# zovoilis-lab/Flye

Hardware: AMD Instinct MI355X
Metric: Gbp reads overlapped/sec (higher is better)
Workload: dtype u64

## Files before the change

flye_amd/csrc/fg_api.hip:

```cpp
#include "fg_ctx.h"
#include "fg_stage.h"
#include <chrono>
#include <cmath>

#include <algorithm>
#include <new>

#include <mutex>
#include <atomic>

static std::mutex g_poolMutex;
static std::vector<BatchOwner*> g_pool;

BatchOwner* BatchOwner::acquire()
{
	std::lock_guard<std::mutex> lock(g_poolMutex);
	if (g_pool.empty()) return new BatchOwner;
	BatchOwner* b = g_pool.back();
	g_pool.pop_back();
	return b;
}

void BatchOwner::release(BatchOwner* b)
{
// ... 39 lines not shown
	}
}

const char* fg_last_error(const fg_ctx* ctx) { return ctx ? ctx->lastError.c_str() : ""; }

int fg_create(fg_ctx** out, int device, int kmer_size)
{
	if (!out) return FG_ERR_ARG;
	*out = nullptr;
	if (kmer_size < 1 || kmer_size > 32) return FG_ERR_KMER_SIZE;
	RandStreamGuard keepCallersRandStream;
	int count = 0;
	if (hipGetDeviceCount(&count) != hipSuccess || count <= 0) return FG_ERR_NO_DEVICE;
	if (device < 0 || device >= count) return FG_ERR_NO_DEVICE;
	if (hipSetDevice(device) != hipSuccess) return FG_ERR_NO_DEVICE;
	fg_ctx* c = new (std::nothrow) fg_ctx;
	if (!c) return FG_ERR_NOMEM;
	c->device = device;
	c->k = kmer_size;
	if (hipStreamCreateWithFlags(&c->stream, hipStreamNonBlocking) != hipSuccess ||
		hipStreamCreateWithFlags(&c->stream2, hipStreamNonBlocking) != hipSuccess ||
		hipStreamCreateWithFlags(&c->stream3, hipStreamNonBlocking) != hipSuccess ||
		hipEventCreateWithFlags(&c->evJoin3, hipEventDisableTiming) != hipSuccess ||
		hipEventCreateWithFlags(&c->evOff, hipEventDisableTiming) != hipSuccess ||
		hipEventCreateWithFlags(&c->evFork, hipEventDisableTiming) != hipSuccess ||
		hipEventCreateWithFlags(&c->evJoin, hipEventDisableTiming) != hipSuccess)
	{
		delete c;
		return FG_ERR_NO_DEVICE;
	}
	for (auto& e : c->evPiece)
		if (hipEventCreateWithFlags(&e, hipEventDisableTiming) != hipSuccess) { delete c; return FG_ERR_NO_DEVICE; }
	c->timer.stream = c->stream;
	*out = c;
	return FG_OK;
}

void fg_destroy(fg_ctx* ctx)
{
	if (!ctx) return;
	(void)hipSetDevice(ctx->device);
	(void)hipStreamSynchronize(ctx->stream);
	delete ctx;
}

int fg_container_info(const fg_ctx* c, uint32_t* first_id, uint32_t* n_fwd, uint32_t* query_first_id, uint32_t* query_n_fwd)
// ... 537 lines not shown
{
	if (!c || !clear_bits || !violations) return FG_ERR_ARG;
	return guarded(c, [&]()
	{
		HIP_CHECK(hipSetDevice(c->device));
		if (!c->indexBuilt) throw FgError{FG_ERR_STATE, "no index"};
		u64 cb = 0, vi = 0;
		fgDebugProbeSkipCheck(c, &cb, &vi);
		*clear_bits = cb; *violations = vi;
	});
}

int fg_debug_chain_lazy(fg_ctx* c, uint64_t out[6])
{
	if (!c || !out) return FG_ERR_ARG;
	return guarded(c, [&]()
	{
		HIP_CHECK(hipSetDevice(c->device));
		u64 h[6];
		fgDebugChainLazy(c, h);
		for (int i = 0; i < 6; ++i) out[i] = h[i];
	});
}

int fg_debug_edit_distances(fg_ctx* c, uint32_t n_pairs, int use_hpc, int32_t* out_dist, int32_t* out_len_a,
							int32_t* out_len_b)
{
	if (!c || (n_pairs && (!out_dist || !out_len_a || !out_len_b))) return FG_ERR_ARG;
	return guarded(c, [&]()
	{
		HIP_CHECK(hipSetDevice(c->device));
		fgDebugEditDistances(c, n_pairs, use_hpc, out_dist, out_len_a, out_len_b);
	});
}

namespace {
struct CigarOwner {
	std::vector<uint64_t> runOff;
	std::vector<uint8_t> ops;
	std::vector<int32_t> lens;
	std::vector<float> err;
};
}

int fg_align_cigar_ksw(fg_ctx* c, uint32_t n_pairs, const uint8_t* trg, const uint64_t* trg_off, const uint8_t* qry,
					   const uint64_t* qry_off, struct fg_cigar_batch* out)
// ... 700 lines not shown
```

flye_amd/csrc/fg_chain.hip:

```cpp
#include "fg_wavesort.h"

#include <algorithm>

#define WG 256
#define I32_MIN ((i32)0x80000000)

struct ChainParams {
	int k, maxJump, minOverlap, maxOverhang;
	int checkOverhang, forceLocal;
	float minUnique;
	u32 firstId;
	u32 qFirstId;
	int onlyMaxExt;
	int keepAln;
	int ablate;
	int lazy;
	unsigned long long* lazyCnt;
};

namespace {

struct CandAcc {
	typedef int4 T;
	int4* c;
// ... 103 lines not shown
	if (!CLASSES)
	{
		append2_multi(a, b, (u32)g0, list, listBig, counts);
		if (fusedMax)
		{
			__syncthreads();
			append2_multi(f, m, (u32)g0, listFused, listFused, counts + 2);
		}
		return;
	}
	u32 oA, oB, oF, oM;
	append2_offsets(a, b, counts, oA, oB);
	__syncthreads();
	append2_offsets(f, m, counts + 2, oF, oM);
#pragma unroll
	for (int t = 0; t < LIST_ITEMS; ++t)
	{
		const u32 g = (u32)g0 + (u32)t;
		if (a[t]) list[(size_t)mid - 1 - oA++] = g;
		if (b[t]) listBig[(size_t)mid - 1 - oB++] = g;
		if (f[t]) listFused[oF++] = g;
		if (m[t]) { list[(size_t)mid + oM] = g; listBig[(size_t)mid + oM] = g; ++oM; }
	}
}

#ifndef FIN_CAP_S
#define FIN_CAP_S 256
#endif
#ifndef FIN_CAP_M
#define FIN_CAP_M 1024
#endif
#ifndef FIN_WAVES_S
#define FIN_WAVES_S 1
#endif
#ifndef FIN_WAVES_G
#define FIN_WAVES_G 1
#endif
#ifndef FIN_BT_CAP
#define FIN_BT_CAP 1024
#endif
__global__ void k_dp_list(u64 nGroups, const u32* __restrict__ dpSize, u32 hugeMin, u32 doneMax ,
						  u32* __restrict__ listSmall, u32* __restrict__ listMid, u32* __restrict__ listBig, u32* __restrict__ counts)
{
	const u64 g0 = ((u64)blockIdx.x * WG + threadIdx.x) * LIST_ITEMS;
	bool a[LIST_ITEMS], b[LIST_ITEMS], h[LIST_ITEMS], none[LIST_ITEMS];
#pragma unroll
// ... 784 lines not shown
}

u32 fgChainSmallMax()
{
	if (getenv("FG_CHAIN_FUSED") && atoi(getenv("FG_CHAIN_FUSED")) == 0) return 0u;
	return getenv("FG_FUSED_CAP") ? (u32)std::max(64, std::min(1024, atoi(getenv("FG_FUSED_CAP")))) : (u32)FIN_CAP_S;
}

void fgChainStage(fg_ctx* c, const fg_detector_params* p, uint8_t forceLocal, u64 nGroups, u64 nHits, int keyMode,
				  int curBits)
{
	hipStream_t s = c->stream;
	ChainParams cp;
	cp.k = c->k; cp.maxJump = p->max_jump; cp.minOverlap = p->min_overlap; cp.maxOverhang = p->max_overhang;
	cp.checkOverhang = p->max_overhang > 0; cp.forceLocal = forceLocal ? 1 : 0;
	cp.minUnique = fgChainMinUnique(p);
	cp.firstId = c->firstId;
	cp.qFirstId = c->hasQ ? c->qFirstId : c->firstId;
	cp.onlyMaxExt = p->only_max_ext ? 1 : 0;
	cp.keepAln = p->keep_alignment ? 1 : 0;
	cp.ablate = getenv("FG_ABLATE") ? atoi(getenv("FG_ABLATE")) : 0;
	cp.lazy = cp.onlyMaxExt && !(getenv("FG_CHAIN_LAZY") && atoi(getenv("FG_CHAIN_LAZY")) == 0);
	cp.lazyCnt = c->dLazyCnt.p;
	if (!nGroups) return;
	const i32* qLen = c->hasQ ? c->dQLen.p : c->dLen.p;
	u32 minSize = 0;
	while ((float)minSize < cp.minUnique) ++minSize;
	if (minSize == 0) minSize = 1;
	const u32 fusedMax = fgChainSmallMax();
	const bool fused = fusedMax != 0;
	const bool classes = fusedMax >= (u32)FIN_CAP_S;
	c->dListBig.reserve((classes ? 2 : 1) * nGroups + 1); c->dListDp.reserve((classes ? 2 : 1) * nGroups + 1);
	if (!classes) c->dListSmall.reserve(nGroups + 1);
	c->dGroupExtSorted.reserve(nGroups + 1);
	c->dListCnt.reserve(4);
	const u64 hitCap = std::max<u64>(nHits, c->hitCapHint);
	c->dCur.reserve(hitCap + 16); c->dExt.reserve(hitCap + 16);
	c->dScore.reserve(hitCap + 16); c->dBack.reserve(hitCap + 16);
	c->dTmp32.reserve(4 * hitCap + 16);
	c->dCand.reserve(hitCap + 1);
	const unsigned gridG = (unsigned)((nGroups + (u64)WG * LIST_ITEMS - 1) / ((u64)WG * LIST_ITEMS));
	if (fused) c->dListFused.reserve(nGroups + 1);
	const char* hugeEnv = getenv("FG_CHAIN_HUGE_MIN");
	HIP_CHECK(hipMemsetAsync(c->dListCnt.p, 0, 16, s));
	{ ScopedK t(c->timer, "k_group_list");
	  if (classes)
		  hipLaunchKernelGGL(k_group_list<true>, gridG, WG, 0, s, nGroups, nHits, c->dGroupStart.p, minSize, c->dGroupFirstCur.p,
							 c->dGroupLastCur.p, (i32)p->min_overlap, c->dListDp.p, c->dListBig.p,
							 hugeEnv ? (u32)atoi(hugeEnv) : (u32)FIN_CAP_M, hugeEnv ? (u32)atoi(hugeEnv) : 4096u, (u32)nGroups,
							 c->dListFused.p, fusedMax, c->dListCnt.p, c->dPrimFlag.p, c->dDpSize.p);
	  else
		  hipLaunchKernelGGL(k_group_list<false>, gridG, WG, 0, s, nGroups, nHits, c->dGroupStart.p, minSize, c->dGroupFirstCur.p,
							 c->dGroupLastCur.p, (i32)p->min_overlap, c->dListSmall.p, c->dListBig.p, (u32)PREP_CAP, 0u, 0u,
							 c->dListFused.p, fusedMax, c->dListCnt.p, c->dPrimFlag.p, c->dDpSize.p); }
	u32 nPrep[4];
	c->hScalar.reserve(8);
	HIP_CHECK(hipMemcpyAsync(c->hScalar.p, c->dListCnt.p, 16, hipMemcpyDeviceToHost, s));
	HIP_CHECK(hipStreamSynchronize(s));
	memcpy(nPrep, c->hScalar.p, 16);
	const u32 nFused = fused ? nPrep[2] : 0u;
	if (!nPrep[0] && !nPrep[1] && !nPrep[3] && !nFused) return;
	const bool sideStreams = !(getenv("FG_CHAIN_STREAMS") && atoi(getenv("FG_CHAIN_STREAMS")) == 1);
	auto launchSmall = [&]()
	{
		if (!nFused) return;
		ScopedK t(c->timer, "k_chain_small");
#define SMALL_ARGS(view) cp, c->dListFused.p, nFused, nGroups, nHits, c->dGroupStart.p, c->dGroupQuery.p, c->curQuery, c->dLen.p, qLen, \
// ... 24 lines not shown
		else if (keyMode == 1)
			hipLaunchKernelGGL(k_group_prep<PK>, gridP, PREP_WAVES * 64, 0, on,
							   PREP_ARGS((HitKeyView<PK>{(const PK*)c->dHitKey.p, nullptr, curBits, c->firstId})));
		else
			hipLaunchKernelGGL(k_group_prep<u64>, gridP, PREP_WAVES * 64, 0, on,
							   PREP_ARGS((HitKeyView<u64>{c->dHitKey.p, c->dHitVal.p, curBits, c->firstId})));
#undef PREP_ARGS
	};
#define FIN_ARGS(list, n) cp, list, n, nGroups, nHits, c->dGroupStart.p, c->dGroupQuery.p, c->curQuery, c->dLen.p, \
		qLen, c->dGroupExt.p, c->dCur.p, c->dExt.p, c->dScore.p, c->dBack.p, c->dTmp32.p, c->dCand.p, c->dPrimFlag.p, c->dDpSize.p
#define DP_ARGS(list, n) cp, list, n, nGroups, nHits, c->dGroupStart.p, c->dGroupQuery.p, c->curQuery, c->dLen.p, qLen, \
		c->dGroupExtSorted.p, c->dDpSize.p, c->dCur.p, c->dExt.p, c->dScore.p, c->dBack.p
	if (classes)
	{
		const bool smallCall = (nPrep[0] + nPrep[1] + nPrep[3] + nFused) < 65536u && !getenv("FG_CHAIN_NO_SMALL_CALL");
		const u32 nMid = nPrep[0] + (smallCall ? 0u : nPrep[3]), nHuge = nPrep[1] + (smallCall ? nPrep[3] : 0u);
		const u32* listMid = c->dListDp.p + (nGroups - nPrep[0]);
		const u32* listHuge = c->dListBig.p + (nGroups - nPrep[1]);
		const bool midLds = smallCall && (!hugeEnv || (u32)atoi(hugeEnv) <= (u32)FIN_CAP_M);
		const bool side = sideStreams && (nMid || nHuge);
		hipStream_t sMid = side ? c->stream2 : s, sHuge = side ? c->stream3 : s;
		const bool split = side && !smallCall && !nHuge && !(getenv("FG_CHAIN_SPLIT") && atoi(getenv("FG_CHAIN_SPLIT")) == 0);
		const u32 nMidB = split ? nMid / 2 : 0u, nMidA = nMid - nMidB;
		auto chain = [&](const u32* list, u32 n, hipStream_t on, bool lds)
		{
			if (!n) return;
			launchPrep(list, n, on);
			{ ScopedK t(c->timer, "k_chain_dp", on);
			  hipLaunchKernelGGL(k_chain_dp, (n + DP_WAVES - 1) / DP_WAVES, DP_WAVES * 64, 0, on, DP_ARGS(list, n)); }
			if (lds)
			{
				ScopedK t(c->timer, "k_chain_finish<lds1024>", on);
				hipLaunchKernelGGL((k_chain_finish<FIN_CAP_M, 1>), n, 64, FIN_CAP_M * 20, on, FIN_ARGS(list, n));
			}
			else
			{
				ScopedK t(c->timer, "k_chain_finish<global>", on);
				hipLaunchKernelGGL((k_chain_finish<0, FIN_WAVES_G, FIN_BT_CAP>), (n + FIN_WAVES_G - 1) / FIN_WAVES_G, FIN_WAVES_G * 64, 0, on,
								   FIN_ARGS(list, n));
			}
		};
		if (side)
		{
			HIP_CHECK(hipEventRecord(c->evFork, s));
			if (nMidA) HIP_CHECK(hipStreamWaitEvent(sMid, c->evFork, 0));
			if (nHuge || nMidB) HIP_CHECK(hipStreamWaitEvent(sHuge, c->evFork, 0));
		}
		chain(listHuge, nHuge, sHuge, false);
		chain(listMid, nMidA, sMid, midLds);
		chain(listMid + nMidA, nMidB, sHuge, midLds);
		launchSmall();
		if (side)
		{
			if (nMidA)
			{
				HIP_CHECK(hipEventRecord(c->evJoin, sMid));
				HIP_CHECK(hipStreamWaitEvent(s, c->evJoin, 0));
			}
			if (nHuge || nMidB)
			{
				HIP_CHECK(hipEventRecord(c->evJoin3, sHuge));
				HIP_CHECK(hipStreamWaitEvent(s, c->evJoin3, 0));
			}
		}
		return;
	}
	launchSmall();
	if (!nPrep[0] && !nPrep[1]) return;
	{
		hipStream_t sBig = s;
		if (sideStreams && nPrep[0] && nPrep[1])
		{
			HIP_CHECK(hipEventRecord(c->evFork, s));
// ... 44 lines not shown
			ScopedK t(c->timer, "k_chain_finish<global>", on);
			hipLaunchKernelGGL((k_chain_finish<0, FIN_WAVES_G, FIN_BT_CAP>), (hc[cls] + FIN_WAVES_G - 1) / FIN_WAVES_G, FIN_WAVES_G * 64, 0, on,
							   FIN_ARGS(lists[cls], hc[cls]));
		}
	}
	if (hc[0])
	{
		{ ScopedK t(c->timer, "k_chain_dp");
		  hipLaunchKernelGGL(k_chain_dp, (hc[0] + DP_WAVES - 1) / DP_WAVES, DP_WAVES * 64, 0, s, DP_ARGS(lists[0], hc[0])); }
		{ ScopedK t(c->timer, "k_chain_finish<lds256>");
		  hipLaunchKernelGGL((k_chain_finish<FIN_CAP_S, FIN_WAVES_S>), (hc[0] + FIN_WAVES_S - 1) / FIN_WAVES_S, FIN_WAVES_S * 64,
							 FIN_CAP_S * 20 * FIN_WAVES_S, s, FIN_ARGS(lists[0], hc[0])); }
	}
	if (side)
	{
		HIP_CHECK(hipEventRecord(c->evJoin, c->stream2));
		HIP_CHECK(hipStreamWaitEvent(s, c->evJoin, 0));
		HIP_CHECK(hipEventRecord(c->evJoin3, c->stream3));
		HIP_CHECK(hipStreamWaitEvent(s, c->evJoin3, 0));
	}
#undef DP_ARGS
#undef FIN_ARGS
}
```

flye_amd/csrc/fg_ctx.h:

```cpp
#pragma once

#include <hip/hip_runtime.h>
#include <cstdint>
#include <cstdio>
#include <cstdlib>
#include <new>
#include <cstring>
#include <string>
#include <vector>
#include <map>
#include <memory>
#include <condition_variable>
#include <functional>
#include <mutex>
#include <thread>
#include <atomic>
#include <algorithm>

#include "../../include/flye_gpu.h"
#include "fg_error.h"

typedef uint64_t u64;
typedef uint32_t u32;
typedef uint16_t u16;
// ... 208 lines not shown
	void run(unsigned n, const std::function<void(unsigned)>& fn)
	{
		if (n <= 1) { fn(0); return; }
		ensure(n);
		std::unique_lock<std::mutex> lk(mu);
		job = &fn; nActive = n; pending = n; ++epoch;
		cvGo.notify_all();
		cvDone.wait(lk, [&] { return pending == 0; });
	}
	~ShimPool()
	{
		{ std::lock_guard<std::mutex> g(mu); stop = true; }
		cvGo.notify_all();
		for (auto& t : threads) if (t.joinable()) t.join();
	}
};

struct fg_ctx {
	int device = 0;
	int k = 17;
	hipStream_t stream = nullptr;
	hipStream_t stream2 = nullptr, stream3 = nullptr;
	hipEvent_t evFork = nullptr, evJoin = nullptr, evJoin3 = nullptr;
#define FG_D2H_MAX_PIECES 16
	hipEvent_t evOff = nullptr, evPiece[FG_D2H_MAX_PIECES] = {};
	unsigned long long pieceEnd[FG_D2H_MAX_PIECES] = {};
	int nPieces = 0;
	std::string lastError;
	KernelTimer timer;

	u32 nReads = 0;
	u32 firstId = 0;
	u64 totalWords = 0, totalBases = 0, totalKmers = 0;
	i32 maxLen = 0;
	std::vector<i32> hLen;
	std::vector<u64> hKmerOff;
	DevBuf<u64> dWords;
	DevBuf<u64> dWordOff;
	DevBuf<i32> dLen;
	DevBuf<u64> dKmerOff;

	bool hasQ = false;
	u32 nQReads = 0, qFirstId = 0;
	i32 qMaxLen = 0;
	std::vector<i32> hQLen;
	DevBuf<u64> dQWords, dQWordOff;
// ... 31 lines not shown
	DevBuf<u64> dPartK0, dPartV0, dPartK1, dPartV1;
	DevBuf<char> dPartScratch;
	DevBuf<unsigned long long> dPartCount;
	DevBuf<u64> dHitOff;
	DevBuf<u64> dFiltOff;
	DevBuf<i32> dFiltPos;
	DevBuf<u64> dHitKey;
	DevBuf<u32> dHitVal;
	DevBuf<u16> dHitVal16;
	bool hitVal16 = false;
	DevBuf<u32> dHitKey32;
	DevBuf<i32> dScore, dBack;
	DevBuf<int4> dCand;
	DevBuf<u64> dGroupStart;
	DevBuf<u32> dGroupQuery;
	DevBuf<u32> dGroupExt, dGroupFirstCur, dGroupLastCur;
	DevBuf<uint8_t> dGroupExtSorted;
	DevBuf<u32> dTmp32;
	DevBuf<fg_seed_hit> dSeedHits;
	DevBuf<u64> dRecvRun, dRecvIdx;
	DevBuf<u32> dRecvErr;
	DevBuf<u64> dCntA, dCntB, dGroupCnt, dGroupOff, dPrimCnt, dPrimOff, dDpGroups, dDpElems;
	DevBuf<u32> dPrimFlag, dDpSize, dListSmall, dListBig, dListDp, dListFused, dListCnt;
	DevBuf<u32> dCur, dExt;
	DevBuf<char> dPrimOut;
	DevBuf<u64> dPrimNode, dPrimBase, dMatchSize, dMatchOff, dMatches;
	DevBuf<u32> dMatchCnt;
	PinnedBuf<u64> hMatches, hMatchOff;
	PinnedBuf<u32> hMatchCnt;
	DevBuf<char> dSortTasks, dSortBig;
	DevBuf<unsigned long long> dSmallElems;
	DevBuf<unsigned long long> dLazyCnt;
	DevBuf<u32> dSortCnt;
	DevBuf<u32> dTieFree;
	u32 tieFreeQ0 = 0, tieFreeN = 0;
	DevBuf<u32> dSortFree, dSortReason;
	u32 sortReasonN = 0;
	u32 sortRadixSegs = 0;
	DevBuf<int> dEditScratch;
	DevBuf<u32> dEditList;
	DevBuf<char> dEditCnt;
	DevBuf<u64> dEditSlab;
	DevBuf<char> dEditPrims;
	DevBuf<u32> dEditQuery;
	DevBuf<i32> dEditOut;
	DevBuf<char> dRangeSides;
// ... 14 lines not shown
	DevBuf<u64> dRcOff, dRcKeys, dRcOut;
	DevBuf<i32> dRcOutScore;
	DevBuf<char> dCovRecs, dCovSort;
	DevBuf<u64> dCovIv, dCovKeys, dCovOff;
	DevBuf<i32> dCovI32, dCovVec;
	DevBuf<char> dPolBytes, dPolCand, dPolItems, dPolTasks, dPolRes;
	DevBuf<u64> dPolOff, dPolEdOff;
	DevBuf<long long> dPolScore, dPolCells, dPolEdits;
	DevBuf<char> dBub[36];
	DevBuf<char> dCc[40];
	DevBuf<char> dCig[20];
	DevBuf<char> dDv[28];
	DevBuf<char> dPt[36];
	PinnedBuf<char> hPrim;
	PinnedBuf<u64> hOff;
	PinnedBuf<u64> hScalar;
	ShimPool shimPool;

	~fg_ctx()
	{
		if (evFork) (void)hipEventDestroy(evFork);
		if (evJoin) (void)hipEventDestroy(evJoin);
		if (evJoin3) (void)hipEventDestroy(evJoin3);
		if (evOff) (void)hipEventDestroy(evOff);
		for (auto e : evPiece) if (e) (void)hipEventDestroy(e);
		if (stream2) (void)hipStreamDestroy(stream2);
		if (stream3) (void)hipStreamDestroy(stream3);
		if (stream) (void)hipStreamDestroy(stream);
	}
};

#if defined(__HIPCC__)

__device__ __forceinline__ i32 fg_uni(i32 v) { return __builtin_amdgcn_readfirstlane(v); }
__device__ __forceinline__ u32 fg_uni(u32 v) { return (u32)__builtin_amdgcn_readfirstlane((int)v); }
__device__ __forceinline__ u64 fg_uni(u64 v)
{
	return ((u64)(u32)__builtin_amdgcn_readfirstlane((int)(u32)(v >> 32)) << 32) |
		   (u32)__builtin_amdgcn_readfirstlane((int)(u32)v);
}

#define FG_PK_VALBITS 24
struct PK {
	u64 v;
	PK() = default;
	__host__ __device__ PK(int x) : v((u64)(unsigned)x) {}
// ... 203 lines not shown
					   float sampleRateInit, u64* histOut);
void fgIndexKmerHist(fg_ctx* c, u64* histOut);
void fgIndexCountSlice(fg_ctx* c, i32 minFreq, float selectRate, i32 tandemFreq, float repeatRate, float sampleRateInit,
					   u32 binLo, u32 binHi, u64* distinctOut, u32* nBatchesOut);
void fgIndexBatchFreq(fg_ctx* c, u32 batch, u32** dFreq, u64* nPos);
void fgIndexBatchSelect(fg_ctx* c, u32 batch);
void fgIndexSelectionDone(fg_ctx* c, u64* histOut);
void fgIndexGatherBegin(fg_ctx* c, u64 nKeys, u64 nEntries, u64 nRep, u64** full, u64** piece, u64* pieceSizes);
void fgIndexGatherEnd(fg_ctx* c, float sampleRate);
void fgIndexBeginMinimizers(fg_ctx* c, i32 minCoverage, i32 window, float repeatRate, u64* histOut);
void fgIndexBuildRange(fg_ctx* c, u32 binLo, u32 binHi, unsigned long long* sumsOut);
void fgIndexFinish(fg_ctx* c, const unsigned long long* totalSums, fg_index_stats* st);
void fgIndexLookupStructures(fg_ctx* c, bool bitsHoldSelection);
void fgImportIndex(fg_ctx* c, u64 nKeys, const u64* keys, const u64* keyOff, u64 nEnt, const u64* entries, u64 nRep,
				   const u64* repKeys, float sampleRate, int onDevice);
u32 fgChainSmallMax();
inline float fgChainMinUnique(const fg_detector_params* p)
{
	const float minKmerSruvivalRate = 0.01;
	return minKmerSruvivalRate * p->min_overlap;
}
void fgChainStage(fg_ctx* c, const fg_detector_params* p, uint8_t forceLocal, u64 nGroups, u64 nHits, int keyMode,
				  int curBits);
void fgEditDistances(fg_ctx* c, PrimRec* dPrims, u64 nPrim, int useHpc);
void fgKswAlign(fg_ctx* c, u32 nPairs, const uint8_t* trg, const u64* trgOff, const uint8_t* qry, const u64* qryOff,
				std::vector<u64>& runOff, std::vector<u32>& runs);
struct FgRangeSide { u32 rec; u32 flags; i32 start, len; };
void fgAlignRanges(fg_ctx* c, const std::vector<FgRangeSide>& sides, bool useHpc, std::vector<u64>& runOff,
				   std::vector<uint8_t>& ops, std::vector<i32>& lens, std::vector<u32>& errBases, std::vector<i32>& lenCur,
				   std::vector<i32>& lenExt);
struct FgDecodedRuns { u32 first, count; const u64* off; u64 nOut; };
void fgAlignRangesDevice(fg_ctx* c, const std::vector<FgRangeSide>& sides, bool useHpc, std::vector<u64>& runOff,
						 std::vector<u32>& errBases, std::vector<i32>& lenCur, std::vector<i32>& lenExt,
						 const std::function<void(const FgDecodedRuns&)>& sink);
void fgTrimRanges(fg_ctx* c, const std::vector<FgRangeSide>& sides, bool useHpc, float maxDivergence, i32 minOverlap,
				  std::vector<u64>& recOff, std::vector<fg_trim_rec>& recs);
void fgSortSegments(fg_ctx* c, const u64* dSegOff, u32 nSeg, u64* dKeys, u32* dVals, u64 n);
void fgEditRanges(fg_ctx* c, const std::vector<FgRangeSide>& sides, bool useHpc, i32* dist, i32* lenCur, i32* lenExt);
struct FgChainAln { i32 curBegin, curEnd, extBegin, extEnd, extLen, score; u32 ext; };
void fgChainAlignments(fg_ctx* c, const fg_chain_params& p, const std::vector<FgChainAln>& tab, const std::vector<u64>& qOff,
					   u64 recBase, const u32* nodeLeft, const u32* nodeRight, u32 nExt, std::vector<u64>& chainOff,
					   std::vector<u64>& alnOff, std::vector<u64>& aln, std::vector<i32>& score);
struct FgCovEdgeEl { i32 extBegin, extEnd; u32 edge, flags; };
void fgReadCoverage(fg_ctx* c, i32 window, i32 maxOverhang, i32 maxFlank, const fg_overlap_rec* recs, const std::vector<u64>& qOff,
					const std::vector<u64>& winOff, const std::vector<i32>& nClip, bool wantVectors, i32* full, i32* junction,
					long long* sum, i32* stat);
// ... 42 lines not shown
```

flye_amd/csrc/fg_overlap.hip:

```cpp
#include "fg_ctx.h"
#include "fg_wavesort.h"
#include "fg_devprim.h"
#include "fg_taskchain.h"
#include <atomic>

#include <algorithm>
#include <cmath>
#include <chrono>
#include <functional>
#include <thread>
#include <type_traits>

#define WG 256
#define FLAG_SELF (1ULL << 63)
#define FLAG_FLIP (1ULL << 62)
#define OFF_MASK ((1ULL << 38) - 1)

namespace {

__device__ __forceinline__ u32 block_exscan(u32 v, u32* sh , u32* total)
{
	const int lane = threadIdx.x & 63, w = threadIdx.x >> 6;
	u32 inc = v;
	for (int o = 1; o < 64; o <<= 1)
// ... 1741 lines not shown
	if (!getenv("FG_KMER_BUDGET") && !getenv("FG_HIT_BUDGET"))
	{
		size_t freeB = 0, totalB = 0;
		HIP_CHECK(hipMemGetInfo(&freeB, &totalB));
		const u64 held = c->dHitKey.bytes() + c->dHitKey32.bytes() + c->dHitVal.bytes() + c->dHitVal16.bytes() + c->dCur.bytes() + c->dExt.bytes() +
						 c->dScore.bytes() + c->dBack.bytes() + c->dTmp32.bytes() + c->dCand.bytes() + c->dProbe.bytes();
		const u64 avail = (u64)freeB + held;
		const u64 usable = avail > (8ULL << 30) ? (avail - (4ULL << 30)) / 10 * 9 : avail / 2;
		hitBudget = std::min(hitBudget, std::max<u64>(16ULL << 20, usable / 100 * 85 / 80));
		kmerBudget = std::min(kmerBudget, std::max<u64>(16ULL << 20, usable / 100 * 15 / 9));
	}
}

static fg_ctx* laneTwo(fg_ctx* c)
{
	if (!c->lane2)
	{
		std::unique_ptr<fg_ctx> l(new fg_ctx);
		l->device = c->device;
		if (hipStreamCreateWithFlags(&l->stream, hipStreamNonBlocking) != hipSuccess ||
			hipStreamCreateWithFlags(&l->stream2, hipStreamNonBlocking) != hipSuccess ||
			hipStreamCreateWithFlags(&l->stream3, hipStreamNonBlocking) != hipSuccess ||
			hipEventCreateWithFlags(&l->evJoin3, hipEventDisableTiming) != hipSuccess ||
			hipEventCreateWithFlags(&l->evOff, hipEventDisableTiming) != hipSuccess ||
			hipEventCreateWithFlags(&l->evFork, hipEventDisableTiming) != hipSuccess ||
			hipEventCreateWithFlags(&l->evJoin, hipEventDisableTiming) != hipSuccess)
			throw FgError{FG_ERR_HIP, "streams of the second lane"};
		for (auto& e : l->evPiece)
			if (hipEventCreateWithFlags(&e, hipEventDisableTiming) != hipSuccess) throw FgError{FG_ERR_HIP, "events of the second lane"};
		l->timer.stream = l->stream;
		c->lane2 = std::move(l);
	}
	fg_ctx* l = c->lane2.get();
	l->k = c->k; l->nReads = c->nReads; l->firstId = c->firstId; l->maxLen = c->maxLen;
	l->totalKmers = c->totalKmers; l->totalBases = c->totalBases;
	l->hasQ = c->hasQ; l->nQReads = c->nQReads; l->qFirstId = c->qFirstId; l->qMaxLen = c->qMaxLen;
	l->indexBuilt = c->indexBuilt; l->sampleRate = c->sampleRate; l->nKeys = c->nKeys; l->nEntries = c->nEntries; l->nRep = c->nRep;
	l->tableSlots = c->tableSlots; l->tableWide = c->tableWide; l->table = c->table;
	l->timer.enabled = c->timer.enabled;
	l->dWords.alias(c->dWords); l->dWordOff.alias(c->dWordOff); l->dLen.alias(c->dLen); l->dKmerOff.alias(c->dKmerOff);
	l->dQWords.alias(c->dQWords); l->dQWordOff.alias(c->dQWordOff); l->dQLen.alias(c->dQLen);
	l->dKeyOff.alias(c->dKeyOff); l->dEntries.alias(c->dEntries); l->dTable.alias(c->dTable); l->dIndexedBits.alias(c->dIndexedBits); l->dMaybeBits.alias(c->dMaybeBits);
	l->dQuery.alias(c->dQuery); l->dQKmerOff.alias(c->dQKmerOff); l->dProbe.alias(c->dProbe);
	l->dCntA.alias(c->dCntA); l->dCntB.alias(c->dCntB);
	l->dLazyCnt.alias(c->dLazyCnt);
	return l;
// ... 476 lines not shown
```

flye_amd/gpu.py:

```python
from __future__ import annotations

import collections
import ctypes as C
import gzip
import os
import random

import time

import numpy as np

_HERE = os.path.dirname(os.path.abspath(__file__))
LIB_PATH = os.environ.get("FLYE_GPU_LIB") or os.path.join(_HERE, "lib", "libflyegpu.so")

REC_DTYPE = np.dtype([("cur_id", "<u4"), ("ext_id", "<u4"), ("cur_begin", "<i4"),
                      ("cur_end", "<i4"), ("cur_len", "<i4"), ("ext_begin", "<i4"),
                      ("ext_end", "<i4"), ("ext_len", "<i4"), ("score", "<i4"),
                      ("seq_divergence", "<f4"), ("chain_length", "<i4"),
                      ("filtered_positions", "<i4"), ("edit_distance", "<i4"),
                      ("hpc_len_cur", "<i4"), ("hpc_len_ext", "<i4")])

ABI_SYMBOLS = ["fg_abi_version", "fg_create", "fg_destroy", "fg_strerror", "fg_last_error",
               "fg_container_info", "fg_set_reads", "fg_set_queries", "fg_build_index_solid", "fg_build_index_minimizers",
               "fg_index_begin_solid", "fg_index_begin_minimizers", "fg_index_build_range", "fg_index_finish",
               "fg_index_kmer_hist", "fg_index_count_slice", "fg_index_batch_freq", "fg_index_batch_select",
               "fg_index_selection_done", "fg_index_gather_begin", "fg_index_gather_end", "fg_memory_stats",
               "fg_import_index", "fg_index_device_arrays", "fg_clear_index", "fg_export_index", "fg_overlaps", "fg_release_batch",
               "fg_kernel_times", "fg_debug_sort_pairs", "fg_debug_edit_distances", "fg_align_cigar_ksw", "fg_release_cigars",
               "fg_align_ranges", "fg_trim_ranges", "fg_release_trims", "fg_edit_ranges", "fg_chain_divergence",
               "fg_chain_alignments", "fg_release_chains",
               "fg_read_coverage", "fg_release_coverage", "fg_coverage_windows", "fg_coverage_verdict",
               "fg_edge_coverage", "fg_release_edge_coverage",
               "fg_subs_matrix_load", "fg_polish_bubbles", "fg_release_polish", "fg_make_bubbles", "fg_release_bubbles",
               "fg_uniform_alignments", "fg_release_uniform", "fg_contig_consensus", "fg_release_consensus",
               "fg_expand_cigars", "fg_release_expand", "fg_cigar_parse", "fg_contig_consensus_cigars", "fg_make_bubbles_cigars",
               "fg_divergence_profile", "fg_release_divergence",
               "fg_confirm_positions", "fg_release_confirm", "fg_classify_reads", "fg_release_classify",
               "fg_index_keep_targets", "fg_index_shard", "fg_probe_hits", "fg_overlaps_from_hits",
               "fg_index_piece_split", "fg_index_scatter_begin", "fg_index_scatter_end", "fg_debug_probe_skip_check",
               "fg_group_create", "fg_group_destroy", "fg_group_size", "fg_group_member", "fg_group_last_error",
               "fg_group_set_reads", "fg_group_set_queries", "fg_group_build_index_solid",
               "fg_group_build_index_minimizers", "fg_group_clear_index", "fg_group_overlaps", "fg_group_stats",
               "fg_group_build_info", "fg_debug_freq_accumulate", "fg_debug_group_bin_cuts", "fg_debug_scan",
               "fg_debug_radix_sort_pairs", "fg_debug_tie_free", "fg_debug_chain_lazy", "fg_debug_sort_screen",
               "fg_debug_order_free", "fg_debug_sort_radix_segments"]

RANGE_PAIR_DTYPE = np.dtype([("cur_id", "<u4"), ("ext_id", "<u4"), ("cur_begin", "<i4"), ("cur_end", "<i4"),
                             ("ext_begin", "<i4"), ("ext_end", "<i4")])

TRIM_REC_DTYPE = np.dtype([("cur_begin", "<i4"), ("cur_end", "<i4"), ("ext_begin", "<i4"), ("ext_end", "<i4"),
                           ("run_start", "<i4"), ("run_end", "<i4"), ("range_err", "<i4"), ("range_len", "<i4"),
                           ("seq_divergence", "<f4")])

SEED_HIT_DTYPE = np.dtype([("cur_pos", "<i4"), ("ext_pos", "<i4"), ("ext_id", "<u4")])


class FlyeGpuError(RuntimeError):
    def __init__(self, code, msg):
        super().__init__(f"libflyegpu error {code}: {msg}")
        self.code = code


class IndexStats(C.Structure):
    _fields_ = [("total_kmers", C.c_uint64), ("selected_kmers", C.c_uint64),
                ("index_entries", C.c_uint64), ("repetitive_kmers", C.c_uint64),
                ("repetitive_frequency", C.c_uint64), ("mean_frequency", C.c_float),
                ("sample_rate", C.c_float), ("build_seconds", C.c_double)]

# ... 227 lines not shown
        L.fg_release_batch.argtypes = [C.POINTER(OverlapBatch)]
        L.fg_index_keep_targets.argtypes = [C.c_void_p, C.c_uint32, C.c_uint32, C.POINTER(C.c_uint64)]
        L.fg_index_shard.argtypes = [C.c_void_p, C.POINTER(C.c_uint32), C.POINTER(C.c_uint32)]
        L.fg_index_piece_split.argtypes = [C.c_void_p, C.c_uint32, C.POINTER(C.c_void_p), C.POINTER(C.c_void_p), C.c_void_p]
        L.fg_index_scatter_begin.argtypes = [C.c_void_p, C.c_uint32, C.c_uint32, C.c_uint64, C.c_uint64, C.c_uint64, C.c_void_p]
        L.fg_index_scatter_end.argtypes = [C.c_void_p, C.c_float]
        L.fg_probe_hits.argtypes = [C.c_void_p, C.c_void_p, C.c_uint32, C.c_void_p, C.POINTER(C.c_void_p),
                                    C.POINTER(C.c_uint64)]
        L.fg_overlaps_from_hits.argtypes = [C.c_void_p, C.POINTER(DetectorParams), C.c_void_p, C.c_uint32, C.c_int32,
                                            C.c_uint8, C.c_uint32, C.c_void_p, C.c_void_p, C.POINTER(OverlapBatch)]
        L.fg_kernel_times.argtypes = [C.c_void_p, C.POINTER(KernelTime), C.c_int]
        L.fg_debug_sort_pairs.argtypes = [C.c_void_p, C.c_void_p, C.c_void_p, C.c_void_p, C.c_uint32]
        L.fg_debug_sort_pairs32.argtypes = [C.c_void_p, C.c_void_p, C.c_void_p, C.c_void_p, C.c_uint32, C.c_int, C.c_int,
                                            C.c_void_p, C.POINTER(C.c_uint64), C.POINTER(C.c_uint64)]
        L.fg_debug_sort_pairs32_val16.argtypes = L.fg_debug_sort_pairs32.argtypes
        L.fg_debug_hit_val16.argtypes = [C.c_void_p, C.POINTER(C.c_uint32)]
        L.fg_debug_tie_free.argtypes = [C.c_void_p, C.c_void_p, C.c_uint32, C.POINTER(C.c_uint32), C.POINTER(C.c_uint32)]
        L.fg_debug_sort_screen.argtypes = [C.c_void_p, C.c_void_p, C.c_void_p, C.c_uint32, C.c_int, C.c_int, C.c_void_p,
                                           C.c_float, C.c_int32, C.c_void_p]
        L.fg_debug_order_free.argtypes = [C.c_void_p, C.c_void_p, C.c_uint32, C.POINTER(C.c_uint32), C.POINTER(C.c_uint32)]
        L.fg_debug_sort_radix_segments.argtypes = [C.c_void_p, C.POINTER(C.c_uint32)]
        L.fg_debug_probe_skip_check.argtypes =[C.c_void_p, C.POINTER(C.c_uint64), C.POINTER(C.c_uint64)]
        L.fg_debug_chain_lazy.argtypes = [C.c_void_p, C.POINTER(C.c_uint64)]
        L.fg_debug_edit_distances.argtypes = [C.c_void_p, C.c_uint32, C.c_int, C.c_void_p, C.c_void_p, C.c_void_p]
        L.fg_align_cigar_ksw.argtypes = [C.c_void_p, C.c_uint32, C.c_void_p, C.c_void_p, C.c_void_p, C.c_void_p,
                                         C.POINTER(CigarBatch)]
        L.fg_release_cigars.argtypes = [C.POINTER(CigarBatch)]
        L.fg_align_ranges.argtypes = [C.c_void_p, C.c_void_p, C.c_uint32, C.c_uint8, C.POINTER(CigarBatch), C.c_void_p,
                                      C.c_void_p]
        L.fg_trim_ranges.argtypes = [C.c_void_p, C.c_void_p, C.c_uint32, C.c_uint8, C.c_float, C.c_int32, C.POINTER(TrimBatch)]
        L.fg_release_trims.argtypes = [C.POINTER(TrimBatch)]
        L.fg_release_trims.restype = None
        L.fg_edit_ranges.argtypes = [C.c_void_p, C.c_void_p, C.c_uint32, C.c_uint8, C.c_void_p, C.c_void_p, C.c_void_p,
                                     C.c_void_p]
        L.fg_chain_divergence.argtypes = [C.c_void_p, C.c_void_p, C.c_void_p, C.c_uint32, C.c_void_p]
        L.fg_chain_alignments.argtypes = [C.c_void_p, C.POINTER(ChainParams), C.c_void_p, C.c_void_p, C.c_uint32, C.c_uint32,
                                          C.c_uint32, C.c_void_p, C.c_void_p, C.POINTER(ChainBatch)]
        L.fg_release_chains.argtypes = [C.POINTER(ChainBatch)]
        L.fg_release_chains.restype = None
        L.fg_read_coverage.argtypes = [C.c_void_p, C.POINTER(CoverageParams), C.c_void_p, C.c_void_p, C.c_uint32, C.c_void_p,
                                       C.POINTER(CoverageBatch)]
        L.fg_release_coverage.argtypes = [C.POINTER(CoverageBatch)]
        L.fg_release_coverage.restype = None
        L.fg_coverage_windows.argtypes = [C.c_int32, C.c_int32, C.c_int32, C.POINTER(C.c_int32), C.POINTER(C.c_int32),
                                          C.POINTER(C.c_uint8)]
        L.fg_coverage_verdict.argtypes = [C.POINTER(CoverageParams), C.c_uint32, C.c_void_p, C.c_void_p, C.c_void_p, C.c_void_p,
# ... 479 lines not shown
                                         int(bool(inclusive)), int(bool(in_place))))
        return out

    def debug_radix_sort_pairs(self, keys, vals, begin_bit, end_bit):
        k = np.ascontiguousarray(keys, np.uint64).copy()
        v = np.ascontiguousarray(vals, np.uint64).copy()
        assert len(k) == len(v)
        passes = C.c_int(-1)
        self._check(self.L.fg_debug_radix_sort_pairs(self.h, k.ctypes.data if len(k) else None,
                                                     v.ctypes.data if len(v) else None, len(k), begin_bit, end_bit,
                                                     C.byref(passes)))
        return k, v, int(passes.value)

    def debug_probe_skip_check(self):
        clear, bad = C.c_uint64(0), C.c_uint64(0)
        self._check(self.L.fg_debug_probe_skip_check(self.h, C.byref(clear), C.byref(bad)))
        return int(clear.value), int(bad.value)

    def debug_chain_lazy(self):
        out = (C.c_uint64 * 6)()
        self._check(self.L.fg_debug_chain_lazy(self.h, out))
        return dict(zip(("entered", "fast", "no_live", "tied_top", "root", "overlap_test"), (int(x) for x in out)))

    def debug_edit_distances(self, n_pairs, use_hpc=False):
        d = np.empty(n_pairs, np.int32)
        la = np.empty(n_pairs, np.int32)
        lb = np.empty(n_pairs, np.int32)
        self._check(self.L.fg_debug_edit_distances(self.h, n_pairs, int(bool(use_hpc)), d.ctypes.data,
                                                   la.ctypes.data, lb.ctypes.data))
        return d, la, lb

    def align_cigar_ksw(self, pairs, arrays=False):
        n = len(pairs)
        trg = np.concatenate([np.asarray(a, np.uint8) for a, _ in pairs]) if n else np.empty(0, np.uint8)
        qry = np.concatenate([np.asarray(b, np.uint8) for _, b in pairs]) if n else np.empty(0, np.uint8)
        toff = np.zeros(n + 1, np.uint64)
        qoff = np.zeros(n + 1, np.uint64)
        toff[1:] = np.cumsum([len(a) for a, _ in pairs])
        qoff[1:] = np.cumsum([len(b) for _, b in pairs])
        trg = np.ascontiguousarray(trg if len(trg) else np.zeros(1, np.uint8))
        qry = np.ascontiguousarray(qry if len(qry) else np.zeros(1, np.uint8))
        b = CigarBatch()
        t0 = time.perf_counter()
        self._check(self.L.fg_align_cigar_ksw(self.h, n, trg.ctypes.data, toff.ctypes.data, qry.ctypes.data,
                                              qoff.ctypes.data, C.byref(b)))
        self.last_align_seconds = time.perf_counter() - t0
# ... 1811 lines not shown
```

include/flye_gpu.h:

```cpp
#ifndef FLYE_GPU_H
#define FLYE_GPU_H

#include <stdint.h>

#ifdef __cplusplus
extern "C" {
#endif

#define FG_ABI_VERSION 4

enum {
	FG_OK = 0,
	FG_ERR_NO_DEVICE = -1,
	FG_ERR_HIP = -2,
	FG_ERR_ARG = -3,
	FG_ERR_STATE = -4,
	FG_ERR_KMER_TOO_FREQUENT = -5,
	FG_ERR_KMER_SIZE = -6,
	FG_ERR_UNSUPPORTED = -7,
	FG_ERR_NOMEM = -8
};

typedef struct fg_ctx fg_ctx;

// ... 181 lines not shown

int fg_debug_tie_free(fg_ctx* ctx, uint32_t* out, uint32_t max_n, uint32_t* first_query, uint32_t* n);

int fg_debug_sort_screen(fg_ctx* ctx, const uint32_t* keys, const uint64_t* seg_off, uint32_t n_seg, int cur_bits,
                         int rec_bits, const uint32_t* tie_free, float min_unique, int32_t min_overlap,
                         uint32_t* out_reason);

int fg_debug_order_free(fg_ctx* ctx, uint32_t* out_reason, uint32_t max_n, uint32_t* first_query, uint32_t* n);

int fg_debug_sort_radix_segments(fg_ctx* ctx, uint32_t* segments);

int fg_debug_group_bin_cuts(const uint64_t* hist, uint32_t world, uint32_t* cuts);

int fg_debug_freq_accumulate(fg_ctx* ctx, uint32_t* dst, const uint32_t* src, uint64_t n);

int fg_debug_scan(fg_ctx* ctx, void* data, uint64_t n, int elem_bytes, int inclusive, int in_place);

int fg_debug_radix_sort_pairs(fg_ctx* ctx, uint64_t* keys, uint64_t* vals, uint64_t n, int begin_bit, int end_bit,
                              int* passes_run);

int fg_debug_probe_skip_check(fg_ctx* ctx, uint64_t* clear_bits, uint64_t* violations);

int fg_debug_chain_lazy(fg_ctx* ctx, uint64_t out[6]);

int fg_debug_edit_distances(fg_ctx* ctx, uint32_t n_pairs, int use_hpc, int32_t* out_dist,
                            int32_t* out_len_a, int32_t* out_len_b);

struct fg_cigar_batch {
	uint32_t  n_pairs;
	uint64_t* run_off;
	uint8_t*  ops;
	int32_t*  lens;
	float*    err_rate;
	void*     owner_;
};
int fg_align_cigar_ksw(fg_ctx* ctx, uint32_t n_pairs, const uint8_t* trg, const uint64_t* trg_off,
                       const uint8_t* qry, const uint64_t* qry_off, struct fg_cigar_batch* out);
void fg_release_cigars(struct fg_cigar_batch* b);

struct fg_range_pair { uint32_t cur_id, ext_id; int32_t cur_begin, cur_end, ext_begin, ext_end; };
int fg_align_ranges(fg_ctx* ctx, const struct fg_range_pair* pairs, uint32_t n_pairs, uint8_t use_hpc,
                    struct fg_cigar_batch* out, int32_t* len_cur, int32_t* len_ext);

struct fg_trim_rec {
	int32_t cur_begin, cur_end, ext_begin, ext_end;
	int32_t run_start, run_end;
// ... 292 lines not shown
```

Baseline: 5.317.

## Order mid and huge chain group lists by descending size before DP

Adds a k_group_order counting-sort kernel that reorders the mid and huge group lists by hit count (largest first), using exact bins for the mid range or log-spaced bins otherwise. When the mid list is split across two streams it interleaves groups so both halves get balanced work, and adds an event so the second stream waits for the ordering. The aim is to cut tail imbalance in the chaining DP kernels by scheduling large groups early. It costs extra histogram/scatter launches, a memset and a buffer per call, plus a new cross-stream dependency.

```diff
diff --git a/flye_amd/csrc/fg_api.hip b/flye_amd/csrc/fg_api.hip
--- a/flye_amd/csrc/fg_api.hip
+++ b/flye_amd/csrc/fg_api.hip
@@ -1,5 +1,6 @@
 #include "fg_ctx.h"
 #include "fg_stage.h"
+#include "fg_chainbin.h"
 #include <chrono>
 #include <cmath>
 
@@ -85,6 +86,7 @@
 		hipStreamCreateWithFlags(&c->stream2, hipStreamNonBlocking) != hipSuccess ||
 		hipStreamCreateWithFlags(&c->stream3, hipStreamNonBlocking) != hipSuccess ||
 		hipEventCreateWithFlags(&c->evJoin3, hipEventDisableTiming) != hipSuccess ||
+		hipEventCreateWithFlags(&c->evOrder, hipEventDisableTiming) != hipSuccess ||
 		hipEventCreateWithFlags(&c->evOff, hipEventDisableTiming) != hipSuccess ||
 		hipEventCreateWithFlags(&c->evFork, hipEventDisableTiming) != hipSuccess ||
 		hipEventCreateWithFlags(&c->evJoin, hipEventDisableTiming) != hipSuccess)
@@ -668,6 +670,18 @@
 		for (int i = 0; i < 6; ++i) out[i] = h[i];
 	});
 }
+
+int fg_debug_chain_lists(fg_ctx* c, uint32_t* out_group, uint32_t* out_size, uint32_t max_n, uint32_t part_n[3], int* ordered)
+{
+	if (!c || !part_n || !ordered || (max_n && (!out_group || !out_size))) return FG_ERR_ARG;
+	return guarded(c, [&]()
+	{
+		HIP_CHECK(hipSetDevice(c->device));
+		fgDebugChainLists(c, out_group, out_size, max_n, part_n, ordered);
+	});
+}
+
+uint32_t fg_debug_chain_size_bin(uint32_t n_hits) { return fgChainSizeBin(n_hits); }
 
 int fg_debug_edit_distances(fg_ctx* c, uint32_t n_pairs, int use_hpc, int32_t* out_dist, int32_t* out_len_a,
 							int32_t* out_len_b)
diff --git a/flye_amd/csrc/fg_chain.hip b/flye_amd/csrc/fg_chain.hip
--- a/flye_amd/csrc/fg_chain.hip
+++ b/flye_amd/csrc/fg_chain.hip
@@ -1,4 +1,5 @@
 #include "fg_wavesort.h"
+#include "fg_chainbin.h"
 
 #include <algorithm>
 
@@ -149,6 +150,89 @@
 		if (f[t]) listFused[oF++] = g;
 		if (m[t]) { list[(size_t)mid + oM] = g; listBig[(size_t)mid + oM] = g; ++oM; }
 	}
+}
+
+#define ORD_ITEMS 4
+#define ORD_BINS_MAX 4096
+enum { ORD_HIST = 0, ORD_SCATTER = 1, ORD_ONE = 2 };
+#define ORD_ONE_MAX (WG * ORD_ITEMS)
+__device__ __forceinline__ u32 list_bin(const u32* __restrict__ list, u32 i, u64 nGroups, u64 nHits,
+										const u64* __restrict__ groupStart, u32 lo, u32& g)
+{
+	g = list[i];
+	const u64 n64 = ((u64)g + 1 < nGroups ? groupStart[(u64)g + 1] : nHits) - groupStart[g];
+	const u32 n = (u32)min(n64, (u64)0xffffffffu);
+	return lo ? min(n - min(n, lo), (u32)ORD_BINS_MAX - 1u) : fgChainSizeBin(n);
+}
+template <int MODE>
+__global__ void __launch_bounds__(WG)
+k_group_order(const u32* __restrict__ list, u32 nList, u64 nGroups, u64 nHits, const u64* __restrict__ groupStart,
+			  u32* __restrict__ cnt, u32* __restrict__ outA, u32* __restrict__ outB, u32 parts, u32 nb, u32 lo)
+{
+	__shared__ u32 hist[ORD_BINS_MAX], base[ORD_BINS_MAX], tsum[WG];
+	for (u32 b = threadIdx.x; b < nb; b += WG) hist[b] = 0;
+	__syncthreads();
+	auto put = [&](u32 pos, u32 g)
+	{
+		if (pos >= nList) return;
+		if (parts == 2) (pos & 1u ? outB : outA)[pos >> 1] = g;
+		else outA[pos] = g;
+	};
+	const u32 per = (nb + WG - 1) / WG, b0 = min(nb, threadIdx.x * per), b1 = min(nb, b0 + per);
+	auto binBases = [&](const u32* h)
+	{
+		u32 own = 0;
+		for (u32 b = b0; b < b1; ++b) own += h[b];
+		tsum[threadIdx.x] = own;
+		__syncthreads();
+		u32 above = 0;
+		for (u32 t = threadIdx.x + 1; t < WG; ++t) above += tsum[t];
+		for (u32 b = b1; b-- > b0;) { base[b] = above; above += h[b]; }
+		__syncthreads();
+	};
+	if (MODE == ORD_ONE)
+	{
+		for (u32 i = threadIdx.x; i < nList; i += WG)
+		{
+			u32 g;
+			atomicAdd(&hist[list_bin(list, i, nGroups, nHits, groupStart, lo, g)], 1u);
+		}
+		__syncthreads();
+		binBases(hist);
+		for (u32 i = threadIdx.x; i < nList; i += WG)
+		{
+			u32 g;
+			const u32 b = list_bin(list, i, nGroups, nHits, groupStart, lo, g);
+			put(base[b] + atomicAdd(&hist[b], 0xffffffffu) - 1u, g);
+		}
+		return;
+	}
+	u32 g[ORD_ITEMS], bin[ORD_ITEMS], rank[ORD_ITEMS];
+	const u32 i0 = blockIdx.x * (WG * ORD_ITEMS) + threadIdx.x;
+#pragma unroll
+	for (int t = 0; t < ORD_ITEMS; ++t)
+	{
+		const u32 i = i0 + (u32)t * WG;
+		bin[t] = nb; g[t] = 0; rank[t] = 0;
+		if (i < nList) bin[t] = list_bin(list, i, nGroups, nHits, groupStart, lo, g[t]);
+	}
+#pragma unroll
+	for (int t = 0; t < ORD_ITEMS; ++t)
+		if (bin[t] < nb) rank[t] = atomicAdd(&hist[bin[t]], 1u);
+	__syncthreads();
+	if (MODE == ORD_HIST)
+	{
+		for (u32 b = b0; b < b1; ++b)
+			if (hist[b]) atomicAdd(&cnt[b], hist[b]);
+		return;
+	}
+	binBases(cnt);
+	for (u32 b = b0; b < b1; ++b)
+		if (hist[b]) base[b] += atomicAdd(&cnt[nb + b], hist[b]);
+	__syncthreads();
+#pragma unroll
+	for (int t = 0; t < ORD_ITEMS; ++t)
+		if (bin[t] < nb) put(base[bin[t]] + rank[t], g[t]);
 }
 
 #ifndef FIN_CAP_S
@@ -979,6 +1063,7 @@
 	cp.ablate = getenv("FG_ABLATE") ? atoi(getenv("FG_ABLATE")) : 0;
 	cp.lazy = cp.onlyMaxExt && !(getenv("FG_CHAIN_LAZY") && atoi(getenv("FG_CHAIN_LAZY")) == 0);
 	cp.lazyCnt = c->dLazyCnt.p;
+	c->chainDbg = {};
 	if (!nGroups) return;
 	const i32* qLen = c->hasQ ? c->dQLen.p : c->dLen.p;
 	u32 minSize = 0;
@@ -1000,6 +1085,12 @@
 	if (fused) c->dListFused.reserve(nGroups + 1);
 	const char* hugeEnv = getenv("FG_CHAIN_HUGE_MIN");
 	HIP_CHECK(hipMemsetAsync(c->dListCnt.p, 0, 16, s));
+	const bool ordered = classes && !(getenv("FG_CHAIN_ORDER") && atoi(getenv("FG_CHAIN_ORDER")) == 0);
+	if (ordered)
+	{
+		c->dListOrd.reserve(nGroups + 1); c->dOrdCnt.reserve(2 * ORD_BINS_MAX + 2 * FG_CHAIN_BINS);
+		HIP_CHECK(hipMemsetAsync(c->dOrdCnt.p, 0, (2 * ORD_BINS_MAX + 2 * FG_CHAIN_BINS) * sizeof(u32), s));
+	}
 	{ ScopedK t(c->timer, "k_group_list");
 	  if (classes)
 		  hipLaunchKernelGGL(k_group_list<true>, gridG, WG, 0, s, nGroups, nHits, c->dGroupStart.p, minSize, c->dGroupFirstCur.p,
@@ -1070,6 +1161,20 @@
 		hipStream_t sMid = side ? c->stream2 : s, sHuge = side ? c->stream3 : s;
 		const bool split = side && !smallCall && !nHuge && !(getenv("FG_CHAIN_SPLIT") && atoi(getenv("FG_CHAIN_SPLIT")) == 0);
 		const u32 nMidB = split ? nMid / 2 : 0u, nMidA = nMid - nMidB;
+		const u32 midLo = fusedMax + 1u, midHi = hugeEnv ? (u32)atoi(hugeEnv) : 4096u;
+		auto orderList = [&](const u32* list, u32 n, u32* cnt, u32* outA, u32* outB, u32 parts, hipStream_t on)
+		{
+			ScopedK t(c->timer, "k_group_order", on);
+			const bool exact = parts == 2 && midHi >= midLo && midHi - midLo < (u32)ORD_BINS_MAX;
+			const u32 nb = exact ? (u32)ORD_BINS_MAX : (u32)FG_CHAIN_BINS, lo = exact ? midLo : 0u;
+#define ORD_ARGS list, n, nGroups, nHits, c->dGroupStart.p, cnt, outA, outB, parts, nb, lo
+			if (n <= ORD_ONE_MAX) { hipLaunchKernelGGL(k_group_order<ORD_ONE>, 1, WG, 0, on, ORD_ARGS); return; }
+			const unsigned gridO = (n + WG * ORD_ITEMS - 1) / (WG * ORD_ITEMS);
+			hipLaunchKernelGGL(k_group_order<ORD_HIST>, gridO, WG, 0, on, ORD_ARGS);
+			hipLaunchKernelGGL(k_group_order<ORD_SCATTER>, gridO, WG, 0, on, ORD_ARGS);
+#undef ORD_ARGS
+		};
+		const u32* partA = listMid, * partB = listMid + nMidA, * partHuge = listHuge;
 		auto chain = [&](const u32* list, u32 n, hipStream_t on, bool lds)
 		{
 			if (!n) return;
@@ -1094,9 +1199,28 @@
 			if (nMidA) HIP_CHECK(hipStreamWaitEvent(sMid, c->evFork, 0));
 			if (nHuge || nMidB) HIP_CHECK(hipStreamWaitEvent(sHuge, c->evFork, 0));
 		}
-		chain(listHuge, nHuge, sHuge, false);
-		chain(listMid, nMidA, sMid, midLds);
-		chain(listMid + nMidA, nMidB, sHuge, midLds);
+		if (ordered && nHuge > 1)
+		{
+			orderList(listHuge, nHuge, c->dOrdCnt.p + 2 * ORD_BINS_MAX, c->dListOrd.p + nMid, nullptr, 1u, sHuge);
+			partHuge = c->dListOrd.p + nMid;
+		}
+		chain(partHuge, nHuge, sHuge, false);
+		if (ordered && nMid > 1)
+		{
+			orderList(listMid, nMid, c->dOrdCnt.p, c->dListOrd.p, c->dListOrd.p + nMidA, nMidB ? 2u : 1u, sMid);
+			partA = c->dListOrd.p; partB = c->dListOrd.p + nMidA;
+			if (nMidB)
+			{
+				HIP_CHECK(hipEventRecord(c->evOrder, sMid));
+				HIP_CHECK(hipStreamWaitEvent(sHuge, c->evOrder, 0));
+			}
+		}
+		chain(partA, nMidA, sMid, midLds);
+		chain(partB, nMidB, sHuge, midLds);
+		c->chainDbg.list[0] = partA; c->chainDbg.n[0] = nMidA;
+		c->chainDbg.list[1] = partB; c->chainDbg.n[1] = nMidB;
+		c->chainDbg.list[2] = partHuge; c->chainDbg.n[2] = nHuge;
+		c->chainDbg.nGroups = nGroups; c->chainDbg.nHits = nHits; c->chainDbg.ordered = ordered ? 1 : 0;
 		launchSmall();
 		if (side)
 		{
@@ -1187,3 +1311,26 @@
 #undef DP_ARGS
 #undef FIN_ARGS
 }
+
+void fgDebugChainLists(fg_ctx* c, u32* outGroup, u32* outSize, u32 maxN, u32 partN[3], int* ordered)
+{
+	const auto& d = c->chainDbg;
+	*ordered = d.ordered;
+	u32 at = 0;
+	for (int i = 0; i < 3; ++i)
+	{
+		partN[i] = d.n[i];
+		const u32 m = std::min(d.n[i], maxN - at);
+		if (m) HIP_CHECK(hipMemcpyAsync(outGroup + at, d.list[i], m * 4ULL, hipMemcpyDeviceToHost, c->stream));
+		at += m;
+	}
+	if (!at) return;
+	std::vector<u64> start(d.nGroups);
+	HIP_CHECK(hipMemcpyAsync(start.data(), c->dGroupStart.p, d.nGroups * 8ULL, hipMemcpyDeviceToHost, c->stream));
+	HIP_CHECK(hipStreamSynchronize(c->stream));
+	for (u32 i = 0; i < at; ++i)
+	{
+		const u64 g = outGroup[i];
+		outSize[i] = (u32)std::min<u64>((g + 1 < d.nGroups ? start[g + 1] : d.nHits) - start[g], 0xffffffffu);
+	}
+}
diff --git a/flye_amd/csrc/fg_chainbin.h b/flye_amd/csrc/fg_chainbin.h
--- /dev/null
+++ b/flye_amd/csrc/fg_chainbin.h
@@ -0,0 +1,16 @@
+#pragma once
+#include <stdint.h>
+
+#if defined(__HIPCC__)
+#define FG_BIN_HD __host__ __device__
+#else
+#define FG_BIN_HD
+#endif
+
+#define FG_CHAIN_BINS 128
+FG_BIN_HD inline uint32_t fgChainSizeBin(uint32_t n)
+{
+	if (n < 4u) return n;
+	const uint32_t e = 31u - (uint32_t)__builtin_clz(n);
+	return 4u * (e - 1u) + ((n >> (e - 2u)) & 3u);
+}
diff --git a/flye_amd/csrc/fg_ctx.h b/flye_amd/csrc/fg_ctx.h
--- a/flye_amd/csrc/fg_ctx.h
+++ b/flye_amd/csrc/fg_ctx.h
@@ -254,6 +254,7 @@
 	hipStream_t stream = nullptr;
 	hipStream_t stream2 = nullptr, stream3 = nullptr;
 	hipEvent_t evFork = nullptr, evJoin = nullptr, evJoin3 = nullptr;
+	hipEvent_t evOrder = nullptr;
 #define FG_D2H_MAX_PIECES 16
 	hipEvent_t evOff = nullptr, evPiece[FG_D2H_MAX_PIECES] = {};
 	unsigned long long pieceEnd[FG_D2H_MAX_PIECES] = {};
@@ -331,6 +332,8 @@
 	DevBuf<u32> dRecvErr;
 	DevBuf<u64> dCntA, dCntB, dGroupCnt, dGroupOff, dPrimCnt, dPrimOff, dDpGroups, dDpElems;
 	DevBuf<u32> dPrimFlag, dDpSize, dListSmall, dListBig, dListDp, dListFused, dListCnt;
+	DevBuf<u32> dListOrd, dOrdCnt;
+	struct ChainListDbg { const u32* list[3] = {nullptr, nullptr, nullptr}; u32 n[3] = {0, 0, 0}; u64 nGroups = 0, nHits = 0; int ordered = 0; } chainDbg;
 	DevBuf<u32> dCur, dExt;
 	DevBuf<char> dPrimOut;
 	DevBuf<u64> dPrimNode, dPrimBase, dMatchSize, dMatchOff, dMatches;
@@ -391,6 +394,7 @@
 		if (evFork) (void)hipEventDestroy(evFork);
 		if (evJoin) (void)hipEventDestroy(evJoin);
 		if (evJoin3) (void)hipEventDestroy(evJoin3);
+		if (evOrder) (void)hipEventDestroy(evOrder);
 		if (evOff) (void)hipEventDestroy(evOff);
 		for (auto e : evPiece) if (e) (void)hipEventDestroy(e);
 		if (stream2) (void)hipStreamDestroy(stream2);
@@ -640,6 +644,7 @@
 }
 void fgChainStage(fg_ctx* c, const fg_detector_params* p, uint8_t forceLocal, u64 nGroups, u64 nHits, int keyMode,
 				  int curBits);
+void fgDebugChainLists(fg_ctx* c, u32* outGroup, u32* outSize, u32 maxN, u32 partN[3], int* ordered);
 void fgEditDistances(fg_ctx* c, PrimRec* dPrims, u64 nPrim, int useHpc);
 void fgKswAlign(fg_ctx* c, u32 nPairs, const uint8_t* trg, const u64* trgOff, const uint8_t* qry, const u64* qryOff,
 				std::vector<u64>& runOff, std::vector<u32>& runs);
diff --git a/flye_amd/csrc/fg_overlap.hip b/flye_amd/csrc/fg_overlap.hip
--- a/flye_amd/csrc/fg_overlap.hip
+++ b/flye_amd/csrc/fg_overlap.hip
@@ -1787,6 +1787,7 @@
 			hipStreamCreateWithFlags(&l->stream2, hipStreamNonBlocking) != hipSuccess ||
 			hipStreamCreateWithFlags(&l->stream3, hipStreamNonBlocking) != hipSuccess ||
 			hipEventCreateWithFlags(&l->evJoin3, hipEventDisableTiming) != hipSuccess ||
+			hipEventCreateWithFlags(&l->evOrder, hipEventDisableTiming) != hipSuccess ||
 			hipEventCreateWithFlags(&l->evOff, hipEventDisableTiming) != hipSuccess ||
 			hipEventCreateWithFlags(&l->evFork, hipEventDisableTiming) != hipSuccess ||
 			hipEventCreateWithFlags(&l->evJoin, hipEventDisableTiming) != hipSuccess)
diff --git a/flye_amd/gpu.py b/flye_amd/gpu.py
--- a/flye_amd/gpu.py
+++ b/flye_amd/gpu.py
@@ -43,7 +43,7 @@
                "fg_group_build_index_minimizers", "fg_group_clear_index", "fg_group_overlaps", "fg_group_stats",
                "fg_group_build_info", "fg_debug_freq_accumulate", "fg_debug_group_bin_cuts", "fg_debug_scan",
                "fg_debug_radix_sort_pairs", "fg_debug_tie_free", "fg_debug_chain_lazy", "fg_debug_sort_screen",
-               "fg_debug_order_free", "fg_debug_sort_radix_segments"]
+               "fg_debug_order_free", "fg_debug_sort_radix_segments", "fg_debug_chain_lists", "fg_debug_chain_size_bin"]
 
 RANGE_PAIR_DTYPE = np.dtype([("cur_id", "<u4"), ("ext_id", "<u4"), ("cur_begin", "<i4"), ("cur_end", "<i4"),
                              ("ext_begin", "<i4"), ("ext_end", "<i4")])
@@ -317,6 +317,10 @@
         L.fg_debug_sort_radix_segments.argtypes = [C.c_void_p, C.POINTER(C.c_uint32)]
         L.fg_debug_probe_skip_check.argtypes =[C.c_void_p, C.POINTER(C.c_uint64), C.POINTER(C.c_uint64)]
         L.fg_debug_chain_lazy.argtypes = [C.c_void_p, C.POINTER(C.c_uint64)]
+        L.fg_debug_chain_lists.argtypes = [C.c_void_p, C.c_void_p, C.c_void_p, C.c_uint32, C.POINTER(C.c_uint32),
+                                           C.POINTER(C.c_int)]
+        L.fg_debug_chain_size_bin.argtypes = [C.c_uint32]
+        L.fg_debug_chain_size_bin.restype = C.c_uint32
         L.fg_debug_edit_distances.argtypes = [C.c_void_p, C.c_uint32, C.c_int, C.c_void_p, C.c_void_p, C.c_void_p]
         L.fg_align_cigar_ksw.argtypes = [C.c_void_p, C.c_uint32, C.c_void_p, C.c_void_p, C.c_void_p, C.c_void_p,
                                          C.POINTER(CigarBatch)]
@@ -842,6 +846,16 @@
         self._check(self.L.fg_debug_chain_lazy(self.h, out))
         return dict(zip(("entered", "fast", "no_live", "tied_top", "root", "overlap_test"), (int(x) for x in out)))
 
+    def debug_chain_lists(self):
+        n = (C.c_uint32 * 3)()
+        flag = C.c_int(0)
+        self._check(self.L.fg_debug_chain_lists(self.h, None, None, 0, n, C.byref(flag)))
+        total = int(sum(n))
+        ids, sizes = np.zeros(max(1, total), np.uint32), np.zeros(max(1, total), np.uint32)
+        self._check(self.L.fg_debug_chain_lists(self.h, ids.ctypes.data, sizes.ctypes.data, total, n, C.byref(flag)))
+        cuts = np.cumsum([0] + [int(x) for x in n])
+        return [(ids[a:b].copy(), sizes[a:b].copy()) for a, b in zip(cuts[:-1], cuts[1:])], bool(flag.value)
+
     def debug_edit_distances(self, n_pairs, use_hpc=False):
         d = np.empty(n_pairs, np.int32)
         la = np.empty(n_pairs, np.int32)
diff --git a/include/flye_gpu.h b/include/flye_gpu.h
--- a/include/flye_gpu.h
+++ b/include/flye_gpu.h
@@ -227,6 +227,11 @@
 int fg_debug_probe_skip_check(fg_ctx* ctx, uint64_t* clear_bits, uint64_t* violations);
 
 int fg_debug_chain_lazy(fg_ctx* ctx, uint64_t out[6]);
+
+int fg_debug_chain_lists(fg_ctx* ctx, uint32_t* out_group, uint32_t* out_size, uint32_t max_n, uint32_t part_n[3],
+                         int* ordered);
+
+uint32_t fg_debug_chain_size_bin(uint32_t n_hits);
 
 int fg_debug_edit_distances(fg_ctx* ctx, uint32_t n_pairs, int use_hpc, int32_t* out_dist,
                             int32_t* out_len_a, int32_t* out_len_b);
```

Result: no change. 5.285 (-0.6%).
